# helemanc/audio-based-lyrics-matching

Measured on NVIDIA B200. Metric: similarity+MAP eval Gpairs/s at 1/2/4/8 B200 (roofline frac); MAP parity, higher is better.
Workload: dtype f16 tensor-core hi/lo split x3, f32 accumulate

## Files before the change

audio-based-lyrics-matching_b200/csrc/api.cu:

```cuda
#include <algorithm>
#include <cstdarg>
#include <cstdio>
#include <cstdlib>
#include <cstring>
#include <functional>
#include <mutex>
#include <vector>

#include <cub/device/device_radix_sort.cuh>
#include <cub/device/device_scan.cuh>
#include <cub/iterator/transform_input_iterator.cuh>

#include "../../include/wealy_b200.h"
#include "epilogues.cuh"
#include "eval_sym_epilogue.cuh"
#include "gemm_core2.cuh"
#include "eval_kernels.cuh"
#include "f64_kernels.cuh"
#include "loss_kernels.cuh"
#include "masked_kernels.cuh"
#include "pool_kernels.cuh"
#include "prep.cuh"
#include "redux_kernels.cuh"
#include "topk_sym_kernels.cuh"
// ... 635 lines not shown
  }
  CU_TRY(cudaGetLastError());
  return WEALY_OK;
}

extern "C" size_t wealy_dot_matrix_backward_workspace_bytes(int64_t n, int64_t m, int64_t d, int passes) {
  if (n <= 0 || m <= 0 || d <= 0) return 0;
  return planes_bytes(n, m, passes) + planes_bytes(m, n, passes) + planes_bytes(d, n, passes) + planes_bytes(d, m, passes) + 8192;
}

extern "C" int wealy_dot_matrix_backward(const void* grad, int64_t ld_grad, const void* grad_t, int64_t ld_grad_t,
                                         const void* xt, int64_t ld_xt, const void* yt, int64_t ld_yt, int64_t n, int64_t m,
                                         int64_t d, int dtype, int passes, void* dx, int64_t ld_dx, void* dy, int64_t ld_dy,
                                         void* workspace, size_t workspace_bytes, void* stream) {
  cudaStream_t s = (cudaStream_t)stream;
  if (n <= 0 || m <= 0 || d <= 0) return fail(WEALY_ERR_BAD_ARG, "bad shape n=%lld m=%lld d=%lld", (long long)n, (long long)m, (long long)d);
  if (!grad || !grad_t || !xt || !yt || !dx || !dy || !workspace) return fail(WEALY_ERR_BAD_ARG, "null pointer");
  if (passes != 1 && passes != 3) return fail(WEALY_ERR_BAD_ARG, "passes must be 1 or 3");
  if (workspace_bytes < wealy_dot_matrix_backward_workspace_bytes(n, m, d, passes)) return fail(WEALY_ERR_WORKSPACE, "workspace too small");
  uint8_t* cur = reinterpret_cast<uint8_t*>(align_up((size_t)workspace, 1024));
  Planes pg, pgt, pxt, pyt;
  carve_planes(pg, cur, n, m, passes);
  carve_planes(pgt, cur, m, n, passes);
  carve_planes(pxt, cur, d, n, passes);
  carve_planes(pyt, cur, d, m, passes);
  W_TRY(launch_prep(grad, ld_grad, n, m, dtype, kPrepRawPow2, 0.f, pg, nullptr, nullptr, 0, nullptr, 0, s));
  W_TRY(launch_prep(grad_t, ld_grad_t, m, n, dtype, kPrepRawPow2, 0.f, pgt, nullptr, nullptr, 0, nullptr, 0, s));
  W_TRY(launch_prep(xt, ld_xt, d, n, dtype, kPrepRawPow2, 0.f, pxt, nullptr, nullptr, 0, nullptr, 0, s));
  W_TRY(launch_prep(yt, ld_yt, d, m, dtype, kPrepRawPow2, 0.f, pyt, nullptr, nullptr, 0, nullptr, 0, s));
  auto product = [&](const Planes& a, const Planes& b, int64_t rows, void* out, int64_t ld_out) -> int {
    StoreParams sp;
    memset(&sp, 0, sizeof(sp));
    sp.out = out;
    sp.ld = ld_out;
    sp.mode = kSimDotsim;
    sp.out_dtype = dtype == WEALY_F32 ? kOutF32 : (dtype == WEALY_F16 ? kOutF16 : kOutBF16);
    sp.post = 1.f;
    sp.rscale = a.scale;
    sp.cscale = b.scale;
    GemmShape sh;
    fill_shape(sh, rows, d, a.d_pad, 64, 1 << 20);
    return launch_gemm<StoreEpi>(passes, a, b, sh, sp, s);
  };
  W_TRY(product(pg, pyt, n, dx, ld_dx));
  W_TRY(product(pgt, pxt, m, dy, ld_dy));
  return WEALY_OK;
}

struct wealy_eval_plan {
  int64_t nq = 0, nc = 0;
  cudaStream_t stream = nullptr;
  cudaStream_t last_stream = nullptr;
  bool same_ids = false;
  int *q_c = nullptr, *q_i = nullptr, *c_c = nullptr, *c_i = nullptr;
  int *sorted_c = nullptr, *sorted_idx = nullptr;
  int *seg_lo = nullptr, *seg_len = nullptr, *npos = nullptr;
  long long* off = nullptr;
  int64_t total_pairs = 0, no_relevant = 0, max_relevant = 0;
  int64_t max_clique = 0;
  float *raw = nullptr, *thr = nullptr, *lim = nullptr;
  int* cnt = nullptr;
  unsigned int* hist = nullptr;
  void* planes_buf = nullptr;
  size_t planes_cap = 0;
  void* topk_buf = nullptr;
  size_t topk_cap = 0;
  void* tks_buf = nullptr;
  size_t tks_cap = 0;
  int last_topk_path = 0;
  int *s_i = nullptr, *s_seg_lo = nullptr, *s_seg_len = nullptr, *s_npos = nullptr;
  long long* s_off = nullptr;
  float4* s_lvl = nullptr;
  void* lvl_thr_buf = nullptr;
  uint2* s_cinfo = nullptr;
  unsigned char* s_dirty = nullptr;
  int64_t s_padded = 0;
  cudaEvent_t ev0 = nullptr, ev1 = nullptr;
  cudaEvent_t evs[4] = {nullptr, nullptr, nullptr, nullptr};
  bool timed = false;
  bool finished = false;
  bool last_sym = false;
  int staged_chunks = 0;
  cudaEvent_t host_ev[1 + 8] = {nullptr, nullptr, nullptr, nullptr, nullptr, nullptr, nullptr, nullptr, nullptr};
  int64_t early_lo = -1, early_ld = 0, early_d = 0;
  const void* early_z = nullptr;
  int early_dtype = 0, early_passes = 0;
  float early_eps = 0.f;
};

static cudaStream_t upload_stream();

extern "C" void wealy_eval_plan_destroy(wealy_eval_plan* p) {
  if (!p) return;
  if (p->early_lo >= 0) {
    cudaStream_t up = upload_stream();
    if (up) cudaStreamSynchronize(up);
  }
  void* ptrs[] = {p->q_c, p->q_i, p->sorted_c, p->sorted_idx, p->seg_lo, p->seg_len, p->npos, p->off,
                  p->raw, p->lvl_thr_buf ? nullptr : (void*)p->thr, p->lim, p->cnt, p->hist,
                  p->s_i, p->s_seg_lo, p->s_seg_len, p->s_npos, p->s_off, p->lvl_thr_buf ? p->lvl_thr_buf : (void*)p->s_lvl,
                  p->s_cinfo, p->s_dirty};
  cudaStream_t fs = p->timed ? p->last_stream : p->stream;
  for (void* q : ptrs) dev_free(q, fs);
  big_free(p->planes_buf, p->planes_cap, fs);
  big_free(p->topk_buf, p->topk_cap, fs);
  big_free(p->tks_buf, p->tks_cap, fs);
  if (!p->same_ids) {
    dev_free(p->c_c, fs);
    dev_free(p->c_i, fs);
  }
  pool_trim();
  if (p->ev0) cudaEventDestroy(p->ev0);
  if (p->ev1) cudaEventDestroy(p->ev1);
  for (cudaEvent_t e : p->evs)
    if (e) cudaEventDestroy(e);
  for (cudaEvent_t e : p->host_ev)
    if (e) cudaEventDestroy(e);
  delete p;
}

struct WidenI32 {
  __host__ __device__ __forceinline__ long long operator()(const int& v) const { return (long long)v; }
};
using WideCounts = cub::TransformInputIterator<long long, WidenI32, const int*>;

static int plan_build(wealy_eval_plan* p, const int64_t* queries_c, const int64_t* queries_i,
                      const int64_t* candidates_c, const int64_t* candidates_i, cudaStream_t s,
                      const std::function<int()>& after_sort = nullptr) {
  const int nq = (int)p->nq, nc = (int)p->nc;
  const int T = 256;
  TempAllocs tmps(s);
  int* bad = nullptr;
  unsigned long long* totals = nullptr;
  CU_TRY(tmps.alloc((void**)&bad, 256));
  totals = reinterpret_cast<unsigned long long*>(bad + 16);
  CU_TRY(cudaMemsetAsync(bad, 0, 256, s));
  CU_TRY(dev_alloc((void**)&p->q_c, (size_t)nq * 4 + 4, s));
  CU_TRY(dev_alloc((void**)&p->q_i, (size_t)nq * 4 + 4, s));
  ids_to_i32_kernel<<<(unsigned)ceil_div(nq, T), T, 0, s>>>((const long long*)queries_c, p->q_c, nq, bad);
  ids_to_i32_kernel<<<(unsigned)ceil_div(nq, T), T, 0, s>>>((const long long*)queries_i, p->q_i, nq, bad);
  p->same_ids = (queries_c == candidates_c && queries_i == candidates_i && p->nq == p->nc);
  if (!p->same_ids && p->nq == p->nc) {
    ids_differ_kernel<<<(unsigned)ceil_div(nq, T), T, 0, s>>>((const long long*)queries_c, (const long long*)queries_i,
                                                             (const long long*)candidates_c, (const long long*)candidates_i, nq, bad + 8);
    int differ = 1;
    CU_TRY(cudaMemcpyAsync(&differ, bad + 8, sizeof(int), cudaMemcpyDeviceToHost, s));
    CU_TRY(cudaStreamSynchronize(s));
    p->same_ids = differ == 0;
  }
  if (p->same_ids) {
    p->c_c = p->q_c;
    p->c_i = p->q_i;
  } else {
    CU_TRY(dev_alloc((void**)&p->c_c, (size_t)nc * 4 + 4, s));
    CU_TRY(dev_alloc((void**)&p->c_i, (size_t)nc * 4 + 4, s));
    ids_to_i32_kernel<<<(unsigned)ceil_div(nc, T), T, 0, s>>>((const long long*)candidates_c, p->c_c, nc, bad);
    ids_to_i32_kernel<<<(unsigned)ceil_div(nc, T), T, 0, s>>>((const long long*)candidates_i, p->c_i, nc, bad);
  }
  CU_TRY(cudaGetLastError());

  int* iota = nullptr;
  CU_TRY(tmps.alloc((void**)&iota, (size_t)nc * 4 + 4));
  CU_TRY(dev_alloc((void**)&p->sorted_c, (size_t)nc * 4 + 4, s));
  CU_TRY(dev_alloc((void**)&p->sorted_idx, (size_t)nc * 4 + 4, s));
  iota_kernel<<<(unsigned)ceil_div(nc, T), T, 0, s>>>(iota, nc);
  size_t tmp_bytes = 0;
  CU_TRY(cub::DeviceRadixSort::SortPairs(nullptr, tmp_bytes, p->c_c, p->sorted_c, iota, p->sorted_idx, nc, 0, 32, s));
  void* tmp = nullptr;
  CU_TRY(tmps.alloc((void**)&tmp, tmp_bytes + 16));
  CU_TRY(cub::DeviceRadixSort::SortPairs(tmp, tmp_bytes, p->c_c, p->sorted_c, iota, p->sorted_idx, nc, 0, 32, s));
  if (after_sort && p->same_ids) W_TRY(after_sort());

  CU_TRY(dev_alloc((void**)&p->seg_lo, (size_t)nq * 4 + 4, s));
  CU_TRY(dev_alloc((void**)&p->seg_len, (size_t)nq * 4 + 4, s));
  CU_TRY(dev_alloc((void**)&p->npos, (size_t)nq * 4 + 4, s));
  CU_TRY(dev_alloc((void**)&p->off, ((size_t)nq + 1) * 8, s));
  segment_lookup_kernel<<<(unsigned)ceil_div(nq, T), T, 0, s>>>(p->q_c, p->q_i, nq, p->sorted_c, p->sorted_idx, p->c_i,
                                                               nc, p->seg_lo, p->seg_len, p->npos, totals);
  CU_TRY(cudaGetLastError());
  size_t scan_bytes = 0;
  CU_TRY(cub::DeviceScan::ExclusiveSum(nullptr, scan_bytes, WideCounts(p->npos, WidenI32()), p->off, nq + 1, s));
  void* tmp2 = nullptr;
  CU_TRY(tmps.alloc((void**)&tmp2, scan_bytes + 16));
  CU_TRY(cudaMemsetAsync(p->npos + nq, 0, 4, s));
  CU_TRY(cub::DeviceScan::ExclusiveSum(tmp2, scan_bytes, WideCounts(p->npos, WidenI32()), p->off, nq + 1, s));

  void* tmp3 = nullptr;
  int *vkeys = nullptr, *vpos = nullptr, *everything = nullptr;
  if (p->same_ids) {
    const int n = nq;
    const int nrb = (int)ceil_div(n, kTileM), nct = (int)ceil_div(n, kTileN);
    p->s_padded = (int64_t)nct * kTileN + kTileN;
    CU_TRY(dev_alloc((void**)&p->s_i, (size_t)n * 4 + 4, s));
    CU_TRY(dev_alloc((void**)&p->s_seg_lo, (size_t)n * 4 + 4, s));
    CU_TRY(dev_alloc((void**)&p->s_seg_len, (size_t)n * 4 + 4, s));
    CU_TRY(dev_alloc((void**)&p->s_npos, (size_t)n * 4 + 4, s));
    CU_TRY(dev_alloc((void**)&p->s_off, ((size_t)n + 1) * 8, s));
    CU_TRY(dev_alloc((void**)&p->s_cinfo, (size_t)p->s_padded * 8, s));
    CU_TRY(dev_alloc((void**)&p->s_dirty, (size_t)nrb * nct, s));
// ... 440 lines not shown
  CU_TRY(cudaEventRecord(p->ev1, s));
  p->timed = true;
  p->finished = finish;

  if (local) {
    CU_TRY(cudaEventRecord(p->evs[2], s));
    topk_sym_local_kernel<<<(unsigned)ceil_div(rows_q * 32, 128), 128, 0, s>>>(tk_val, tk_idx, tk_cnt, tk_cap2, (int)rows_q, (int)nq,
                                                                              topk, p->sorted_idx, topk_sim, local_idx, local_cnt);
    CU_TRY(cudaGetLastError());
    CU_TRY(cudaEventRecord(p->evs[3], s));
    p->finished = true;
    return WEALY_OK;
  }

  if (finish) {
    const int threads = 256;
    const unsigned blocks = (unsigned)ceil_div(nq * 32, threads);
    if (sym) ap_reduce_kernel<<<blocks, threads, 0, s>>>(p->hist, p->s_off, p->cnt, (int)nq, aps, r1s, sums, p->sorted_idx);
    else ap_reduce_kernel<<<blocks, threads, 0, s>>>(p->hist, p->off, p->cnt, (int)nq, aps, r1s, sums);
    CU_TRY(cudaGetLastError());
    CU_TRY(cudaEventRecord(p->evs[2], s));
    if (sym_topk) {
      topk_sym_finalize_kernel<<<(unsigned)ceil_div(rows_q * 32, 128), 128, 0, s>>>(tk_val, tk_idx, tk_cnt, tk_cap2, (int)rows_q, (int)nq,
                                                                                   topk, p->sorted_idx, (long long*)topk_idx, topk_sim,
                                                                                   tk_fail);
      CU_TRY(cudaGetLastError());
      CU_TRY(cudaEventRecord(p->evs[3], s));
      int failed = 0;
      CU_TRY(cudaMemcpyAsync(&failed, tk_fail, 4, cudaMemcpyDeviceToHost, s));
      CU_TRY(cudaStreamSynchronize(s));
      if (failed != 0) {
        W_TRY(eval_run_impl(p, queries_z, ld_q, candidates_z, ld_c, d, dtype, eps, passes, topk, aps, r1s, sums, topk_idx, topk_sim,
                            shard_rank, shard_world, finish, stream, chunks, redux, q_len, c_len, false));
        p->last_topk_path = 3;
      }
      return WEALY_OK;
    }
    if (topk > 0) {
      if (parts * cap <= 32 * kFinPerLane) {
        float* stage_val = reinterpret_cast<float*>(ep.cand_cnt + (size_t)parts * nq);
        int* stage_idx = reinterpret_cast<int*>(stage_val + (size_t)parts * nq * cap);
        topk_finalize_select_kernel<<<(unsigned)ceil_div(nq * 32, 128), 128, 0, s>>>(
            ep.cand_val, ep.cand_idx, ep.cand_cnt, parts, (int)nq, cap, topk, stage_val, stage_idx,
            (long long*)topk_idx, topk_sim);
      } else {
        topk_finalize_kernel<<<blocks, threads, 0, s>>>(ep.cand_val, ep.cand_idx, ep.cand_cnt, parts, (int)nq, cap, topk,
                                                        (long long*)topk_idx, topk_sim);
      }
      CU_TRY(cudaGetLastError());
    }
    CU_TRY(cudaEventRecord(p->evs[3], s));
  }
  return WEALY_OK;
}

extern "C" int wealy_eval_plan_last_topk_path(const wealy_eval_plan* p, int* path) {
  if (!p || !path) return fail(WEALY_ERR_BAD_ARG, "null pointer");
  *path = p->last_topk_path;
  return WEALY_OK;
}

extern "C" int wealy_eval_plan_stage_ms(const wealy_eval_plan* p, float* ms) {
  if (!p || !ms) return fail(WEALY_ERR_BAD_ARG, "null pointer");
  if (!p->timed) return fail(WEALY_ERR_BAD_ARG, "the plan has not been run yet");
  CU_TRY(cudaEventSynchronize(p->finished ? p->evs[3] : p->ev1));
  CU_TRY(cudaEventElapsedTime(&ms[0], p->evs[0], p->evs[1]));
  CU_TRY(cudaEventElapsedTime(&ms[1], p->evs[1], p->ev0));
  CU_TRY(cudaEventElapsedTime(&ms[2], p->ev0, p->ev1));
  ms[3] = ms[4] = 0.f;
  if (p->finished) {
    CU_TRY(cudaEventElapsedTime(&ms[3], p->ev1, p->evs[2]));
    CU_TRY(cudaEventElapsedTime(&ms[4], p->evs[2], p->evs[3]));
  }
  return WEALY_OK;
}

extern "C" int wealy_eval_run(wealy_eval_plan* p, const void* queries_z, int64_t ld_q, const void* candidates_z,
                              int64_t ld_c, int64_t d, int dtype, float eps, int passes, int topk, float* aps,
                              float* r1s, double* sums, int64_t* topk_idx, float* topk_sim, void* stream) {
  return eval_run_impl(p, queries_z, ld_q, candidates_z, ld_c, d, dtype, eps, passes, topk, aps, r1s, sums, topk_idx,
                       topk_sim, 0, 1, true, stream);
}

static cudaStream_t upload_stream() {
  static cudaStream_t streams[64] = {nullptr};
  static std::mutex mu;
  int dev = 0;
  cudaGetDevice(&dev);
  if (dev < 0 || dev >= 64) return nullptr;
  std::lock_guard<std::mutex> lock(mu);
  if (!streams[dev] && cudaStreamCreateWithFlags(&streams[dev], cudaStreamNonBlocking) != cudaSuccess) streams[dev] = nullptr;
  return streams[dev];
}

template <int kLevels, int kPasses, int kBlockK>
static int launch_sym_part(const Planes& pq, const GemmShape& sh, const EvalSymParams& sp, cudaStream_t s, int max_pairs) {
  return launch_gemm_pair<EvalSymEpi<kLevels>, kPasses, kBlockK, 12, true>(pq, sh, sp, s, nullptr, max_pairs);
}

struct HostUpload {
  const void* z = nullptr;
  int64_t ld = 0, d = 0;
  int dtype = 0;
  float eps = 0.f;
  int up_sms = 0, grid = 0, threads = 0;
  size_t smem = 0;
  cudaStream_t up = nullptr;
};

static int host_upload_setup(HostUpload& h, const void* host_z, int64_t ld, int64_t d, int dtype, float eps, bool* on_device) {
  *on_device = false;
  if (dtype != WEALY_F32 && dtype != WEALY_F16 && dtype != WEALY_BF16) return fail(WEALY_ERR_BAD_ARG, "unknown element type %d", dtype);
  cudaPointerAttributes attr;
  if (cudaPointerGetAttributes(&attr, host_z) != cudaSuccess) {
    cudaGetLastError();
    return fail(WEALY_ERR_UNSUPPORTED, "cannot classify the embeddings' pointer");
  }
  if (attr.type == cudaMemoryTypeDevice || attr.type == cudaMemoryTypeManaged) {
    *on_device = true;
    return WEALY_OK;
  }
  if (d <= 0 || d > 128 * kRowVecs || d % 4 != 0 || ld % 4 != 0 || ld < d)
    return fail(WEALY_ERR_UNSUPPORTED, "wealy_eval_run_host needs rows of 4 k <= %d elements (d=%lld, ld=%lld)", 128 * kRowVecs,
                (long long)d, (long long)ld);
  if (attr.type != cudaMemoryTypeHost || !attr.devicePointer)
    return fail(WEALY_ERR_UNSUPPORTED, "host embeddings must be pinned (page-locked and mapped) to be read by the device");
  h.z = attr.devicePointer;
  if ((reinterpret_cast<uintptr_t>(h.z) & 15) != 0) return fail(WEALY_ERR_UNSUPPORTED, "host embeddings must be 16-byte aligned");
  h.ld = ld;
  h.d = d;
  h.dtype = dtype;
  h.eps = eps;
  h.up = upload_stream();
  if (!h.up) return fail(WEALY_ERR_CUDA, "no upload stream");
  h.up_sms = std::min(std::max(env_int("WEALY_HOST_UP_SMS", 8), 0), num_sms() / 2);
  h.smem = h.up_sms > 0 ? 120 * 1024 : 0;
  h.grid = h.up_sms > 0 ? h.up_sms : num_sms() * std::max(1, env_int("WEALY_HOST_UP_GRID", 1));
  if (h.up_sms > 0) {
    h.threads = std::min(512, std::max(32, env_int("WEALY_HOST_UP_THREADS", 512) / 32 * 32));
  } else {
    h.threads = env_int("WEALY_HOST_UP_THREADS", 64) <= 32 ? 32 : 64;
  }
  const void* up_kernel =
      h.up_sms > 0 ? (dtype == WEALY_F32 ? (const void*)prep_rows_stream_kernel<float, 512>
                      : dtype == WEALY_F16 ? (const void*)prep_rows_stream_kernel<__half, 512>
                                           : (const void*)prep_rows_stream_kernel<__nv_bfloat16, 512>)
                   : (dtype == WEALY_F32 ? (const void*)prep_rows_stream_kernel<float, 64>
                      : dtype == WEALY_F16 ? (const void*)prep_rows_stream_kernel<__half, 64>
                                           : (const void*)prep_rows_stream_kernel<__nv_bfloat16, 64>);
  CU_TRY(cudaFuncSetAttribute(up_kernel, cudaFuncAttributePreferredSharedMemoryCarveout, cudaSharedmemCarveoutMaxShared));
  if (h.smem) CU_TRY(cudaFuncSetAttribute(up_kernel, cudaFuncAttributeMaxDynamicSharedMemorySize, (int)h.smem));
  return WEALY_OK;
}

static int host_upload_rows(const HostUpload& h, const Planes& pq, const int* sorted_idx, int64_t n, int64_t lo, int64_t hi) {
  if (hi <= lo) return WEALY_OK;
#define STREAM_ARGS (long long)h.ld, (int)lo, (int)hi, (int)h.d, (int)pq.d_pad, h.eps, pq.hi, pq.lo, pq.norm, pq.scale, pq.sq, sorted_idx, (int)n
#define STREAM_LAUNCH(T)                                                                                                     \
  do {                                                                                                                       \
    if (h.up_sms > 0) prep_rows_stream_kernel<T, 512><<<h.grid, h.threads, h.smem, h.up>>>((const T*)h.z, STREAM_ARGS);       \
    else prep_rows_stream_kernel<T, 64><<<h.grid, h.threads, 0, h.up>>>((const T*)h.z, STREAM_ARGS);                          \
  } while (0)
  switch (h.dtype) {
    case WEALY_F32: STREAM_LAUNCH(float); break;
    case WEALY_F16: STREAM_LAUNCH(__half); break;
    default: STREAM_LAUNCH(__nv_bfloat16); break;
  }
#undef STREAM_LAUNCH
#undef STREAM_ARGS
  CU_TRY(cudaGetLastError());
  return WEALY_OK;
}

static int host_planes(wealy_eval_plan* p, int64_t d, int passes, cudaStream_t s, Planes& pq) {
  const int64_t rows_q = ceil_div(p->nq, kTileM) * kTileM;
  const size_t need = planes_bytes(rows_q, d, passes) + 2048;
  if (need > p->planes_cap) {
    big_free(p->planes_buf, p->planes_cap, s);
    p->planes_buf = nullptr;
    p->planes_cap = 0;
    CU_TRY(big_alloc((void**)&p->planes_buf, &p->planes_cap, need, s));
  }
  uint8_t* cur = reinterpret_cast<uint8_t*>(align_up((size_t)p->planes_buf, 1024));
  carve_planes(pq, cur, rows_q, d, passes);
  if (!p->ev0) {
    CU_TRY(cudaEventCreate(&p->ev0));
    CU_TRY(cudaEventCreate(&p->ev1));
    for (cudaEvent_t& e : p->evs) CU_TRY(cudaEventCreate(&e));
  }
  for (cudaEvent_t& e : p->host_ev)
    if (!e) CU_TRY(cudaEventCreateWithFlags(&e, cudaEventDisableTiming));
  return WEALY_OK;
}

static float kHostCum[5][8] = {{1.f}, {0.30f, 1.f}, {0.10f, 0.20f, 0.35f, 0.55f, 1.f}, {0.06f, 0.14f, 0.24f, 0.36f, 0.5f, 0.7f, 1.f}, {1.f}};
static int kHostCount[5] = {1, 2, 5, 7, 1};
static int host_preset(int64_t n) {
  const int nsb = (int)ceil_div(n, 2 * kTileM);
  int preset = nsb >= 96 ? 2 : (nsb >= 24 ? 1 : 0);
  const int forced = env_int("WEALY_HOST_PARTS", 0);
  if (forced > 0) preset = forced >= 7 ? 3 : (forced >= 5 ? 2 : (forced >= 2 ? 1 : 0));
  if (const char* cum = getenv("WEALY_HOST_CUM")) {
    static std::mutex mu;
    std::lock_guard<std::mutex> lock(mu);
    int cnt = 0;
    float last = 0.f;
    for (const char* q = cum; *q && cnt < 7;) {
      char* end = nullptr;
      const float v = strtof(q, &end);
      if (end == q) break;
      if (v > last && v < 1.f) kHostCum[4][cnt++] = last = v;
      q = *end == ',' ? end + 1 : end;
      if (*end != ',' && *end != 0) break;
    }
    kHostCum[4][cnt++] = 1.f;
    kHostCount[4] = cnt;
    preset = 4;
  }
  return preset;
}
static int host_part_begin(int64_t n, int preset, int k) {
  const int nsb = (int)ceil_div(n, 2 * kTileM);
  if (k + 1 >= kHostCount[preset]) return 0;
  const int sb = nsb - (int)lroundf(kHostCum[preset][k] * (float)nsb);
  return sb < 0 ? 0 : sb;
}

extern "C" int wealy_eval_plan_create_host(const int64_t* queries_c, const int64_t* queries_i, int64_t nq,
                                           const int64_t* candidates_c, const int64_t* candidates_i, int64_t nc,
                                           const void* host_z, int64_t ld, int64_t d, int dtype, float eps, int passes,
                                           void* stream, wealy_eval_plan** plan) {
  if (!plan) return fail(WEALY_ERR_BAD_ARG, "plan output pointer is null");
  *plan = nullptr;
  if (nq <= 0 || nc <= 0) return fail(WEALY_ERR_BAD_ARG, "empty query or candidate set (nq=%lld nc=%lld)", (long long)nq, (long long)nc);
  if (!queries_c || !queries_i || !candidates_c || !candidates_i) return fail(WEALY_ERR_BAD_ARG, "null id pointer");
  if (nq >= (1ll << 31) - 256 || nc >= (1ll << 31) - 256) return fail(WEALY_ERR_UNSUPPORTED, "more than 2^31 rows");
  cudaStream_t s = (cudaStream_t)stream;
  wealy_eval_plan* p = new wealy_eval_plan();
  p->nq = nq;
  p->nc = nc;
  p->stream = s;
  auto early = [&]() -> int {
    HostUpload h;
    bool on_device = false;
    if (!host_z || (passes != 1 && passes != 3) || env_int("WEALY_HOST_EARLY", 1) == 0) return WEALY_OK;
    if (host_upload_setup(h, host_z, ld, d, dtype, eps, &on_device) != WEALY_OK || on_device) return WEALY_OK;
    Planes pq;
    W_TRY(host_planes(p, d, passes, s, pq));
    const int64_t lo = (int64_t)host_part_begin(nq, host_preset(nq), 0) * 2 * kTileM;
    CU_TRY(cudaEventRecord(p->host_ev[0], s));
    CU_TRY(cudaStreamWaitEvent(h.up, p->host_ev[0], 0));
    W_TRY(host_upload_rows(h, pq, p->sorted_idx, nq, lo, pq.rows));
    p->early_lo = lo;
    p->early_z = h.z;
    p->early_ld = ld;
    p->early_d = d;
    p->early_dtype = dtype;
    p->early_passes = passes;
    p->early_eps = eps;
    return WEALY_OK;
  };
  int st = plan_build(p, queries_c, queries_i, candidates_c, candidates_i, s, early);
  if (st != WEALY_OK) {
    wealy_eval_plan_destroy(p);
    return st;
  }
  *plan = p;
  return WEALY_OK;
}

extern "C" int wealy_eval_run_host(wealy_eval_plan* p, const void* host_z, int64_t ld, int64_t d, int dtype, float eps,
                                   int passes, float* aps, float* r1s, double* sums, void* stream) {
  cudaStream_t s = (cudaStream_t)stream;
  if (!p || !host_z || !aps || !r1s || !sums) return fail(WEALY_ERR_BAD_ARG, "null pointer");
  if (passes != 1 && passes != 3) return fail(WEALY_ERR_BAD_ARG, "passes must be 1 or 3");
  const int64_t n = p->nq;
  if (!(p->same_ids && p->nq == p->nc && p->total_pairs < (1ll << 31) - 8))
    return fail(WEALY_ERR_UNSUPPORTED, "wealy_eval_run_host evaluates all-vs-all plans (queries == candidates)");
  HostUpload h;
  bool on_device = false;
  W_TRY(host_upload_setup(h, host_z, ld, d, dtype, eps, &on_device));
  if (on_device)
    return eval_run_impl(p, host_z, ld, host_z, ld, d, dtype, eps, passes, 0, aps, r1s, sums, nullptr, nullptr, 0, 1, true, stream);
  const void* z = h.z;
  cudaStream_t up = h.up;
  const int up_sms = h.up_sms;
  const void* kpos_kernels[2] = {(const void*)pos_pairs_sorted_kernel<false>, (const void*)pos_sort_sorted_kernel};
  struct RestoreCarveout {
    const void* const* k;
    bool on;
    ~RestoreCarveout() {
      for (int i = 0; on && i < 2; ++i) cudaFuncSetAttribute(k[i], cudaFuncAttributePreferredSharedMemoryCarveout, cudaSharedmemCarveoutDefault);
    }
  } restore{kpos_kernels, up_sms == 0};
  if (up_sms == 0)
    for (const void* k : kpos_kernels)
      CU_TRY(cudaFuncSetAttribute(k, cudaFuncAttributePreferredSharedMemoryCarveout, cudaSharedmemCarveoutMaxShared));

  Planes pq;
  W_TRY(host_planes(p, d, passes, s, pq));
  const int64_t rows_q = pq.rows;
  int64_t early_lo = -1;
  if (p->early_lo >= 0 && p->early_z == z && p->early_ld == ld && p->early_d == d && p->early_dtype == dtype &&
      p->early_passes == passes && p->early_eps == eps)
    early_lo = p->early_lo;
  p->early_lo = -1;

  const int nsb = (int)ceil_div(n, 2 * kTileM);
  const int preset = host_preset(n);
  const int n_parts = kHostCount[preset];
  const int64_t reach = p->max_clique > 1 ? p->max_clique : 1;

  GemmShape sh0;
  fill_shape(sh0, n, n, pq.d_pad, 64, 1 << 20, env_int("WEALY_TILES_PER_UNIT", 8));
  const int total_rb = sh0.n_row_blocks;
  sh0.sym = 1 | (env_int("WEALY_PAIR_INTERLEAVE", 1) != 0 ? 2 : 0);
  if (passes == 3) sh0.k_blocks = (int)(pq.d_pad / 32);
  EvalSymParams sp;
  memset(&sp, 0, sizeof(sp));
  sp.lvl = p->s_lvl;
  sp.cinfo = p->s_cinfo;
  sp.s_c = p->sorted_c;
  sp.s_i = p->s_i;
  sp.thr = p->thr;
  sp.hist = p->hist;
  sp.dirty = p->s_dirty;
  sp.n_col_tiles = sh0.n_col_tiles;
  sp.n_row_blocks = total_rb;
  sp.total_pairs = (unsigned)p->total_pairs;

  CU_TRY(cudaEventRecord(p->evs[0], s));
  CU_TRY(cudaEventRecord(p->evs[1], s));
  CU_TRY(cudaMemsetAsync(p->hist, 0, (size_t)(p->total_pairs > 0 ? p->total_pairs : 1) * 4, s));
  CU_TRY(cudaMemsetAsync(p->cnt, 0, (size_t)n * 4, s));
  CU_TRY(cudaMemsetAsync(sums, 0, 3 * sizeof(double), s));
  CU_TRY(cudaEventRecord(p->host_ev[0], s));
  CU_TRY(cudaStreamWaitEvent(up, p->host_ev[0], 0));
  CU_TRY(cudaEventRecord(p->ev0, s));

  const bool trace = env_int("WEALY_HOST_TRACE", 0) != 0;
  std::vector<cudaEvent_t> tev;
  auto stamp = [&](cudaStream_t st) {
    if (!trace) return;
    cudaEvent_t e = nullptr;
    cudaEventCreate(&e);
    cudaEventRecord(e, st);
    tev.push_back(e);
  };
  stamp(s);
  int sb_hi = nsb;
  int64_t prep_hi = rows_q;
  for (int k = 0; k < n_parts; ++k) {
    int sb_lo = host_part_begin(n, preset, k);
    if (sb_lo > sb_hi) sb_lo = sb_hi;
    int64_t prep_lo = k + 1 == n_parts ? 0 : ((int64_t)sb_lo * 2 * kTileM - reach) / kTileM * kTileM;
    if (prep_lo < 0) prep_lo = 0;
    if (prep_lo > prep_hi) prep_lo = prep_hi;
    stamp(up);
    W_TRY(host_upload_rows(h, pq, p->sorted_idx, n, prep_lo, early_lo >= 0 ? std::min(prep_hi, early_lo) : prep_hi));
    if (trace) fprintf(stderr, "[wealy host run] part %d: rows [%lld, %lld) arrive, super row blocks [%d, %d) swept\n", k,
                       (long long)prep_lo, (long long)prep_hi, sb_lo, sb_hi);
    prep_hi = prep_lo;
    stamp(up);
    CU_TRY(cudaEventRecord(p->host_ev[1 + k], up));
    CU_TRY(cudaStreamWaitEvent(s, p->host_ev[1 + k], 0));
    stamp(s);
    const int q_lo = sb_lo * 2 * kTileM;
    const int q_hi = (int)std::min<int64_t>((int64_t)sb_hi * 2 * kTileM, n);
    if (q_hi > q_lo) {
      const int threads = 256;
      pos_pairs_sorted_kernel<false><<<(unsigned)ceil_div(q_hi - q_lo, 16), threads, 0, s>>>(
          pq.hi, pq.lo, (int)pq.d_pad, p->sorted_c, p->s_i, (int)n, p->s_seg_lo, p->s_seg_len, p->s_off, p->raw, p->cnt, nullptr,
          q_lo, q_hi);
      const int64_t sort_end = k == 0 ? p->s_padded : q_hi;
      pos_sort_sorted_kernel<<<(unsigned)ceil_div((sort_end - q_lo) * 32, threads), threads, 0, s>>>(
          p->s_npos, (int)n, (int)p->s_padded, p->s_off, p->raw, p->thr, p->cnt, p->s_lvl, p->s_cinfo, q_lo, q_hi, 1);
      CU_TRY(cudaGetLastError());
      stamp(s);
      GemmShape sh = sh0;
      sh.n_row_blocks = sb_hi - sb_lo;
      sh.rb_offset = sb_lo;
      sh.rb_stride = 1;
      sh.group_rows = std::max(1, std::min(num_sms() / 4, sh.n_row_blocks));
      const int max_pairs = (up_sms > 0 && k + 1 < n_parts) ? (num_sms() - up_sms) / 2 : 0;
      if (passes == 3) W_TRY((launch_sym_part<4, 3, 32>(pq, sh, sp, s, max_pairs)));
      else W_TRY((launch_sym_part<3, 1, 64>(pq, sh, sp, s, max_pairs)));
    }
    else stamp(s);
    stamp(s);
    sb_hi = sb_lo;
  }
  CU_TRY(cudaEventRecord(p->ev1, s));
  if (trace) {
    cudaStreamSynchronize(s);
    cudaStreamSynchronize(up);
    for (int k = 0; k < n_parts && (size_t)(1 + 5 * k + 4) < tev.size(); ++k) {
      float t[5];
      for (int j = 0; j < 5; ++j) cudaEventElapsedTime(&t[j], tev[0], tev[1 + 5 * k + j]);
      fprintf(stderr, "[wealy host run] part %d: upload %.3f -> %.3f ms | ready %.3f, K_pos done %.3f, sweep done %.3f ms\n", k, t[0],
              t[1], t[2], t[3], t[4]);
    }
    for (cudaEvent_t e : tev) cudaEventDestroy(e);
  }
  p->timed = true;
  p->finished = true;
  p->last_sym = true;
  p->last_stream = s;
  p->last_topk_path = 0;
  ap_reduce_kernel<<<(unsigned)ceil_div(n * 32, 256), 256, 0, s>>>(p->hist, p->s_off, p->cnt, (int)n, aps, r1s, sums, p->sorted_idx);
  CU_TRY(cudaGetLastError());
  CU_TRY(cudaEventRecord(p->evs[2], s));
  CU_TRY(cudaEventRecord(p->evs[3], s));
  return WEALY_OK;
}

extern "C" int wealy_eval_run_chunked(wealy_eval_plan* p, const void* queries_z, int64_t ld_q, const void* candidates_z,
                                      int64_t ld_c, int64_t d, int dtype, float eps, int passes, int topk, int chunks,
                                      int redux, float* aps, float* r1s, double* sums, int64_t* topk_idx, float* topk_sim,
                                      void* stream) {
  return eval_run_impl(p, queries_z, ld_q, candidates_z, ld_c, d, dtype, eps, passes, topk, aps, r1s, sums, topk_idx,
                       topk_sim, 0, 1, true, stream, chunks, redux);
}

extern "C" int wealy_eval_run_ragged(wealy_eval_plan* p, const void* queries_z, int64_t ld_q, const void* candidates_z,
                                     int64_t ld_c, int64_t d, int dtype, float eps, int passes, int topk, int chunks,
                                     int redux, const int32_t* q_len, const int32_t* c_len, float* aps, float* r1s,
                                     double* sums, int64_t* topk_idx, float* topk_sim, void* stream) {
  if (!q_len || !c_len) return fail(WEALY_ERR_BAD_ARG, "null chunk counts");
  return eval_run_impl(p, queries_z, ld_q, candidates_z, ld_c, d, dtype, eps, passes, topk, aps, r1s, sums, topk_idx,
                       topk_sim, 0, 1, true, stream, chunks, redux, q_len, c_len);
}

extern "C" int wealy_eval_shard_prepare(wealy_eval_plan* p, const void* z, int64_t ld, int64_t d, int dtype, float eps,
                                        int passes, int shard_rank, int shard_world, void* stream) {
  if (shard_world < 2) return fail(WEALY_ERR_BAD_ARG, "staged sweeps are for two or more ranks");
  return eval_run_impl(p, z, ld, z, ld, d, dtype, eps, passes, 0, nullptr, nullptr, nullptr, nullptr, nullptr, shard_rank,
                       shard_world, false, stream, 1, WEALY_REDUX_MIN, nullptr, nullptr, true, 1);
}

extern "C" int wealy_eval_plan_thresholds(const wealy_eval_plan* p, void** values, int64_t* count) {
  if (!p || !values || !count) return fail(WEALY_ERR_BAD_ARG, "null pointer");
  if (!p->lvl_thr_buf) return fail(WEALY_ERR_BAD_ARG, "the plan is not an all-vs-all plan");
  if (p->staged_chunks > 1) {
    *values = p->thr;
    *count = p->total_pairs > 0 ? p->total_pairs : 1;
    return WEALY_OK;
  }
  *values = p->lvl_thr_buf;
  *count = p->s_padded * 4 + (p->total_pairs > 0 ? p->total_pairs : 1);
  return WEALY_OK;
}

static int check_shard_tracks(const wealy_eval_plan* p, int chunks, int shard_rank, int shard_world) {
  if (!p) return fail(WEALY_ERR_BAD_ARG, "null plan");
  if (!p->same_ids) return fail(WEALY_ERR_BAD_ARG, "a sharded sweep needs queries == candidates (ids and embeddings) and no top-k");
  if (chunks != 2 && chunks != 4 && chunks != 8 && chunks != 16)
    return fail(WEALY_ERR_UNSUPPORTED, "chunked tracks have 2, 4, 8 or 16 chunks, got %d", chunks);
  if (shard_world < 1 || shard_rank < 0 || shard_rank >= shard_world) return fail(WEALY_ERR_BAD_ARG, "bad shard %d/%d", shard_rank, shard_world);
  return WEALY_OK;
}

extern "C" int wealy_eval_sweep_shard_tracks(wealy_eval_plan* p, const void* z, int64_t ld, int64_t d, int dtype, float eps,
                                             int passes, int chunks, int redux, const int32_t* lens, int shard_rank,
                                             int shard_world, void* stream) {
  W_TRY(check_shard_tracks(p, chunks, shard_rank, shard_world));
  return eval_run_impl(p, z, ld, z, ld, d, dtype, eps, passes, 0, nullptr, nullptr, nullptr, nullptr, nullptr, shard_rank,
                       shard_world, false, stream, chunks, redux, lens, lens);
}

extern "C" int wealy_eval_shard_prepare_tracks(wealy_eval_plan* p, const void* z, int64_t ld, int64_t d, int dtype, float eps,
                                               int passes, int chunks, int redux, const int32_t* lens, int shard_rank,
                                               int shard_world, void* stream) {
  W_TRY(check_shard_tracks(p, chunks, shard_rank, shard_world));
  if (shard_world < 2) return fail(WEALY_ERR_BAD_ARG, "staged sweeps are for two or more ranks");
  return eval_run_impl(p, z, ld, z, ld, d, dtype, eps, passes, 0, nullptr, nullptr, nullptr, nullptr, nullptr, shard_rank,
                       shard_world, false, stream, chunks, redux, lens, lens, true, 1);
}

extern "C" int wealy_eval_shard_sweep_tracks(wealy_eval_plan* p, int64_t d, int passes, int chunks, int redux,
                                             const int32_t* lens, int shard_rank, int shard_world, void* stream) {
  W_TRY(check_shard_tracks(p, chunks, shard_rank, shard_world));
  if (shard_world < 2) return fail(WEALY_ERR_BAD_ARG, "staged sweeps are for two or more ranks");
  return eval_run_impl(p, nullptr, 0, nullptr, 0, d, WEALY_F32, 0.f, passes, 0, nullptr, nullptr, nullptr, nullptr, nullptr,
// ... 316 lines not shown
```

Before: 438.9.

## Run K_pos kernels on a high-priority side stream to overlap with sweep

```diff
diff --git a/audio-based-lyrics-matching_b200/csrc/api.cu b/audio-based-lyrics-matching_b200/csrc/api.cu
--- a/audio-based-lyrics-matching_b200/csrc/api.cu
+++ b/audio-based-lyrics-matching_b200/csrc/api.cu
@@ -741,6 +741,7 @@
   bool last_sym = false;
   int staged_chunks = 0;
   cudaEvent_t host_ev[1 + 8] = {nullptr, nullptr, nullptr, nullptr, nullptr, nullptr, nullptr, nullptr, nullptr};
+  cudaEvent_t kpos_ev[8] = {nullptr, nullptr, nullptr, nullptr, nullptr, nullptr, nullptr, nullptr};
   int64_t early_lo = -1, early_ld = 0, early_d = 0;
   const void* early_z = nullptr;
   int early_dtype = 0, early_passes = 0;
@@ -774,6 +775,8 @@
   for (cudaEvent_t e : p->evs)
     if (e) cudaEventDestroy(e);
   for (cudaEvent_t e : p->host_ev)
+    if (e) cudaEventDestroy(e);
+  for (cudaEvent_t e : p->kpos_ev)
     if (e) cudaEventDestroy(e);
   delete p;
 }
@@ -1380,16 +1383,23 @@
                        topk_sim, 0, 1, true, stream);
 }
 
-static cudaStream_t upload_stream() {
-  static cudaStream_t streams[64] = {nullptr};
+static cudaStream_t lib_stream(int which) {
+  static cudaStream_t streams[64][2] = {};
   static std::mutex mu;
   int dev = 0;
   cudaGetDevice(&dev);
   if (dev < 0 || dev >= 64) return nullptr;
   std::lock_guard<std::mutex> lock(mu);
-  if (!streams[dev] && cudaStreamCreateWithFlags(&streams[dev], cudaStreamNonBlocking) != cudaSuccess) streams[dev] = nullptr;
-  return streams[dev];
-}
+  cudaStream_t& st = streams[dev][which];
+  if (!st) {
+    int lo = 0, hi = 0;
+    if (which == 1) cudaDeviceGetStreamPriorityRange(&lo, &hi);
+    if (cudaStreamCreateWithPriority(&st, cudaStreamNonBlocking, which == 1 ? hi : 0) != cudaSuccess) st = nullptr;
+  }
+  return st;
+}
+static cudaStream_t upload_stream() { return lib_stream(0); }
+static cudaStream_t kpos_stream() { return lib_stream(1); }
 
 template <int kLevels, int kPasses, int kBlockK>
 static int launch_sym_part(const Planes& pq, const GemmShape& sh, const EvalSymParams& sp, cudaStream_t s, int max_pairs) {
@@ -1487,6 +1497,8 @@
     for (cudaEvent_t& e : p->evs) CU_TRY(cudaEventCreate(&e));
   }
   for (cudaEvent_t& e : p->host_ev)
+    if (!e) CU_TRY(cudaEventCreateWithFlags(&e, cudaEventDisableTiming));
+  for (cudaEvent_t& e : p->kpos_ev)
     if (!e) CU_TRY(cudaEventCreateWithFlags(&e, cudaEventDisableTiming));
   return WEALY_OK;
 }
@@ -1583,17 +1595,17 @@
   const void* z = h.z;
   cudaStream_t up = h.up;
   const int up_sms = h.up_sms;
+  cudaStream_t kp = kpos_stream();
+  if (!kp) return fail(WEALY_ERR_CUDA, "no K_pos stream");
   const void* kpos_kernels[2] = {(const void*)pos_pairs_sorted_kernel<false>, (const void*)pos_sort_sorted_kernel};
   struct RestoreCarveout {
     const void* const* k;
-    bool on;
     ~RestoreCarveout() {
-      for (int i = 0; on && i < 2; ++i) cudaFuncSetAttribute(k[i], cudaFuncAttributePreferredSharedMemoryCarveout, cudaSharedmemCarveoutDefault);
+      for (int i = 0; i < 2; ++i) cudaFuncSetAttribute(k[i], cudaFuncAttributePreferredSharedMemoryCarveout, cudaSharedmemCarveoutDefault);
     }
-  } restore{kpos_kernels, up_sms == 0};
-  if (up_sms == 0)
-    for (const void* k : kpos_kernels)
-      CU_TRY(cudaFuncSetAttribute(k, cudaFuncAttributePreferredSharedMemoryCarveout, cudaSharedmemCarveoutMaxShared));
+  } restore{kpos_kernels};
+  for (const void* k : kpos_kernels)
+    CU_TRY(cudaFuncSetAttribute(k, cudaFuncAttributePreferredSharedMemoryCarveout, cudaSharedmemCarveoutMaxShared));
 
   Planes pq;
   W_TRY(host_planes(p, d, passes, s, pq));
@@ -1632,8 +1644,14 @@
   CU_TRY(cudaMemsetAsync(p->hist, 0, (size_t)(p->total_pairs > 0 ? p->total_pairs : 1) * 4, s));
   CU_TRY(cudaMemsetAsync(p->cnt, 0, (size_t)n * 4, s));
   CU_TRY(cudaMemsetAsync(sums, 0, 3 * sizeof(double), s));
+  if (p->s_padded > n) {
+    pos_sort_sorted_kernel<<<(unsigned)ceil_div((p->s_padded - n) * 32, 256), 256, 0, s>>>(
+        p->s_npos, (int)n, (int)p->s_padded, p->s_off, p->raw, p->thr, p->cnt, p->s_lvl, p->s_cinfo, (int)n, (int)n, 1);
+    CU_TRY(cudaGetLastError());
+  }
   CU_TRY(cudaEventRecord(p->host_ev[0], s));
   CU_TRY(cudaStreamWaitEvent(up, p->host_ev[0], 0));
+  CU_TRY(cudaStreamWaitEvent(kp, p->host_ev[0], 0));
   CU_TRY(cudaEventRecord(p->ev0, s));
 
   const bool trace = env_int("WEALY_HOST_TRACE", 0) != 0;
@@ -1649,9 +1667,10 @@
   int sb_hi = nsb;
   int64_t prep_hi = rows_q;
   for (int k = 0; k < n_parts; ++k) {
+    const bool last = k + 1 == n_parts;
     int sb_lo = host_part_begin(n, preset, k);
     if (sb_lo > sb_hi) sb_lo = sb_hi;
-    int64_t prep_lo = k + 1 == n_parts ? 0 : ((int64_t)sb_lo * 2 * kTileM - reach) / kTileM * kTileM;
+    int64_t prep_lo = last ? 0 : ((int64_t)sb_lo * 2 * kTileM - reach) / kTileM * kTileM;
     if (prep_lo < 0) prep_lo = 0;
     if (prep_lo > prep_hi) prep_lo = prep_hi;
     stamp(up);
@@ -1661,42 +1680,49 @@
     prep_hi = prep_lo;
     stamp(up);
     CU_TRY(cudaEventRecord(p->host_ev[1 + k], up));
-    CU_TRY(cudaStreamWaitEvent(s, p->host_ev[1 + k], 0));
-    stamp(s);
+    CU_TRY(cudaStreamWaitEvent(kp, p->host_ev[1 + k], 0));
+    stamp(kp);
     const int q_lo = sb_lo * 2 * kTileM;
     const int q_hi = (int)std::min<int64_t>((int64_t)sb_hi * 2 * kTileM, n);
     if (q_hi > q_lo) {
       const int threads = 256;
-      pos_pairs_sorted_kernel<false><<<(unsigned)ceil_div(q_hi - q_lo, 16), threads, 0, s>>>(
+      pos_pairs_sorted_kernel<false><<<(unsigned)ceil_div(q_hi - q_lo, 16), threads, 0, kp>>>(
           pq.hi, pq.lo, (int)pq.d_pad, p->sorted_c, p->s_i, (int)n, p->s_seg_lo, p->s_seg_len, p->s_off, p->raw, p->cnt, nullptr,
           q_lo, q_hi);
-      const int64_t sort_end = k == 0 ? p->s_padded : q_hi;
-      pos_sort_sorted_kernel<<<(unsigned)ceil_div((sort_end - q_lo) * 32, threads), threads, 0, s>>>(
+      pos_sort_sorted_kernel<<<(unsigned)ceil_div((q_hi - q_lo) * 32, threads), threads, 0, kp>>>(
           p->s_npos, (int)n, (int)p->s_padded, p->s_off, p->raw, p->thr, p->cnt, p->s_lvl, p->s_cinfo, q_lo, q_hi, 1);
       CU_TRY(cudaGetLastError());
-      stamp(s);
+    }
+    stamp(kp);
+    cudaStream_t ss = last ? kp : s;
+    if (!last) {
+      CU_TRY(cudaEventRecord(p->kpos_ev[k], kp));
+      CU_TRY(cudaStreamWaitEvent(s, p->kpos_ev[k], 0));
+    }
+    stamp(ss);
+    if (q_hi > q_lo) {
       GemmShape sh = sh0;
       sh.n_row_blocks = sb_hi - sb_lo;
       sh.rb_offset = sb_lo;
       sh.rb_stride = 1;
       sh.group_rows = std::max(1, std::min(num_sms() / 4, sh.n_row_blocks));
-      const int max_pairs = (up_sms > 0 && k + 1 < n_parts) ? (num_sms() - up_sms) / 2 : 0;
-      if (passes == 3) W_TRY((launch_sym_part<4, 3, 32>(pq, sh, sp, s, max_pairs)));
-      else W_TRY((launch_sym_part<3, 1, 64>(pq, sh, sp, s, max_pairs)));
+      const int max_pairs = (up_sms > 0 && !last) ? (num_sms() - up_sms) / 2 : 0;
+      if (passes == 3) W_TRY((launch_sym_part<4, 3, 32>(pq, sh, sp, ss, max_pairs)));
+      else W_TRY((launch_sym_part<3, 1, 64>(pq, sh, sp, ss, max_pairs)));
     }
-    else stamp(s);
-    stamp(s);
+    stamp(ss);
     sb_hi = sb_lo;
   }
+  CU_TRY(cudaEventRecord(p->kpos_ev[n_parts - 1], kp));
+  CU_TRY(cudaStreamWaitEvent(s, p->kpos_ev[n_parts - 1], 0));
   CU_TRY(cudaEventRecord(p->ev1, s));
   if (trace) {
     cudaStreamSynchronize(s);
-    cudaStreamSynchronize(up);
-    for (int k = 0; k < n_parts && (size_t)(1 + 5 * k + 4) < tev.size(); ++k) {
-      float t[5];
-      for (int j = 0; j < 5; ++j) cudaEventElapsedTime(&t[j], tev[0], tev[1 + 5 * k + j]);
-      fprintf(stderr, "[wealy host run] part %d: upload %.3f -> %.3f ms | ready %.3f, K_pos done %.3f, sweep done %.3f ms\n", k, t[0],
-              t[1], t[2], t[3], t[4]);
+    for (int k = 0; k < n_parts && (size_t)(1 + 6 * k + 5) < tev.size(); ++k) {
+      float t[6];
+      for (int j = 0; j < 6; ++j) cudaEventElapsedTime(&t[j], tev[0], tev[1 + 6 * k + j]);
+      fprintf(stderr, "[wealy host run] part %d: upload %.3f -> %.3f ms | K_pos %.3f -> %.3f ms | sweep %.3f -> %.3f ms\n", k,
+              t[0], t[1], t[2], t[3], t[4], t[5]);
     }
     for (cudaEvent_t e : tev) cudaEventDestroy(e);
   }
```

Measured after the change: 439.5 (median of 6 runs). No clear change (+0.1%).
